# iamwinter/UMPR

Hardware: AMD Instinct MI355X
Metric: training samples/sec (higher is better)
Workload: dtype f32

## Files before the change

### include/umpr_hip.h

```cpp
#ifndef UMPR_HIP_H
#define UMPR_HIP_H
#include <stddef.h>
#include <stdint.h>

#ifdef __cplusplus
extern "C" {
#endif

const char* umpr_version(void);
const char* umpr_last_error(void);
int umpr_device_info(int dev, char* name, int name_len, int* compute_units, size_t* hbm_bytes);

int umpr_gemm_f32(const float* A, long lda, int transA, const float* B, long ldb, int transB, float* C, long ldc,
                  int M, int N, int K, const float* bias, int bias_mode, int act, int accumulate, float alpha,
                  float* ws, size_t ws_bytes, void* stream);

int umpr_set_gemm_bf16(int on);

int umpr_set_conv_inference(int on);

int umpr_set_conv_pool_follows(int on);

long umpr_debug_wino_fix_count(void);

size_t umpr_embed_gru_bidir_ws_bytes(int N, int L, int E);
int umpr_embed_gru_bidir_fwd(const int64_t* ids, const float* emb, int E,
                             const float* w_ih_f, const float* w_hh_f, const float* b_ih_f, const float* b_hh_f,
                             const float* w_ih_r, const float* w_hh_r, const float* b_ih_r, const float* b_hh_r,
                             const int32_t* lengths, const int32_t* order, const int32_t* dst_row, int N, int L,
                             float* out, float* saved, float* ws, size_t ws_bytes, void* stream);
int umpr_embed_gru_bidir_bwd(const int64_t* ids, const float* emb, int E,
                             const float* w_hh_f, const float* w_hh_r,
                             const int32_t* lengths, const int32_t* order, const int32_t* dst_row, int N, int L,
                             const float* dout, const float* out, const float* saved,
                             float* dw_ih_f, float* dw_hh_f, float* db_ih_f, float* db_hh_f,
                             float* dw_ih_r, float* dw_hh_r, float* db_ih_r, float* db_hh_r,
                             float* ws, size_t ws_bytes, void* stream);

int umpr_embed_gru_bidir_bwd_acc(const int64_t* ids, const float* emb, int E,
                                 const float* w_hh_f, const float* w_hh_r,
                                 const int32_t* lengths, const int32_t* order, const int32_t* dst_row, int N, int L,
                                 const float* dout, const float* out, const float* saved,
                                 float* dw_ih_f, float* dw_hh_f, float* db_ih_f, float* db_hh_f,
                                 float* dw_ih_r, float* dw_hh_r, float* db_ih_r, float* db_hh_r,
                                 int accumulate, float* ws, size_t ws_bytes, void* stream);

size_t umpr_coattention_fwd_ws_bytes(int B, int SL);
int umpr_coattention_fwd(const float* Gu, const float* Gi, const float* M, int B, int SL, float* T, float* soft_u,
                         float* soft_i, float* atte_u, long ld_u, float* atte_i, long ld_i, float* colmax,
                         int32_t* argcol, float* rowmax, int32_t* argrow, float* ws, size_t ws_bytes, void* stream);
int umpr_coattention_fwd_bf16(const float* Gu, const float* Gi, const float* M, int B, int SL, float* T, float* soft_u,
                              float* soft_i, float* atte_u, long ld_u, float* atte_i, long ld_i, float* colmax,
                              int32_t* argcol, float* rowmax, int32_t* argrow, float* ws, size_t ws_bytes, void* stream);
size_t umpr_coattention_bwd_ws_bytes(int B, int SL);
int umpr_coattention_bwd(const float* Gu, const float* Gi, const float* M, const float* T, const float* soft_u,
                         const float* soft_i, const float* colmax, const int32_t* argcol, const float* rowmax,
// ... 190 lines not shown
```

### umpr_amd/_lib.py

```python
from __future__ import annotations

import ctypes
import os
import threading

import torch

_HERE = os.path.dirname(os.path.abspath(__file__))
LIB_PATH = os.path.join(_HERE, "libumpr_hip.so")

_T = {"p": ctypes.c_void_p, "i": ctypes.c_int, "l": ctypes.c_long, "z": ctypes.c_size_t, "f": ctypes.c_float,
      "d": ctypes.c_double, "u": ctypes.c_uint64}

SIGNATURES = {
    "umpr_version": ("", "s"),
    "umpr_last_error": ("", "s"),
    "umpr_device_info": ("ipipp", "i"),
    "umpr_gemm_f32": ("pliplipliiipiiifpzp", "i"),
    "umpr_embed_gru_bidir_ws_bytes": ("iii", "z"),
    "umpr_embed_gru_bidir_fwd": ("ppipppppppppppiipppzp", "i"),
    "umpr_embed_gru_bidir_bwd": ("ppipppppiippppppppppppzp", "i"),
    "umpr_embed_gru_bidir_bwd_acc": ("ppipppppiipppppppppppipzp", "i"),
    "umpr_coattention_fwd_ws_bytes": ("ii", "z"),
    "umpr_coattention_fwd": ("pppiipppplplpppppzp", "i"),
# ... 51 lines not shown
    "umpr_vgg16_cls_arena_bytes": ("i", "z"),
    "umpr_vgg16_classifier_fwd_compact": ("piiiuppppzp", "i"),
    "umpr_vgg16_classifier_bwd_compact": ("piippppppzp", "i"),
    "umpr_vgg16_classifier_fwd_compact_bf16": ("piiiuppppzp", "i"),
    "umpr_vgg16_classifier_bwd_compact_bf16": ("piippppppzp", "i"),
    "umpr_concat_ids": ("pplpp", "i"),
    "umpr_review_net_arena_bytes": ("iii", "z"),
    "umpr_review_net_ws_bytes": ("iiii", "z"),
    "umpr_review_net_fwd": ("ppipppiiiiiipppzp", "i"),
    "umpr_review_net_bwd": ("ppipppiiiippppzp", "i"),
    "umpr_control_net_arena_bytes": ("iiiiiii", "z"),
    "umpr_control_net_ws_bytes": ("iiiiiiiii", "z"),
    "umpr_control_net_fwd": ("pppipppppiiiiiiiifiippppppzp", "i"),
    "umpr_control_net_bwd": ("pppipppppiiiiiiiiipppppppzp", "i"),
    "umpr_head_fwd": ("pppppppppppppfiiipppppppp", "i"),
    "umpr_head_bwd": ("pppppppppppfiiippppppppppppppppppppp", "i"),
    "umpr_photo_resize_u8": ("pzpiiipp", "i"),
    "umpr_photo_store_slot_bytes": ("ii", "z"),
    "umpr_photo_fetch_u8": ("pzpppiiiplpp", "i"),
    "umpr_bce_head_fwd": ("plpppiipppzp", "i"),
    "umpr_bce_head_bwd": ("plpppppiiplpppzp", "i"),
    "umpr_adam_step": ("ppppldddddldp", "i"),
    "umpr_sq_err_accumulate": ("pplpp", "i"),
    "umpr_adam_step_dev": ("pppplddd" "pp", "i"),
    "umpr_grad_norm_ws_bytes": ("", "z"),
    "umpr_grad_norm": ("ppidfppzpp", "i"),
    "umpr_adam_step_clip": ("ppppldddddld" "pp", "i"),
    "umpr_adam_step_dev_clip": ("pppplddd" "ppp", "i"),
    "umpr_debug_poison_lds": ("pp", "i"),
    "umpr_set_gemm_bf16": ("i", "i"),
    "umpr_set_conv_inference": ("i", "i"),
    "umpr_set_conv_pool_follows": ("i", "i"),
    "umpr_debug_wino_fix_count": ("", "l"),
    "umpr_profile_enable": ("i", "i"),
    "umpr_profile_reset": ("", "i"),
    "umpr_profile_read": ("ippp", "i"),
}


class UmprHipError(RuntimeError):
    pass


class _Tls(threading.local):
    gemm_b16 = False


TLS = _Tls()


class _Lib:
    def __init__(self):
        if not os.path.exists(LIB_PATH):
            raise UmprHipError(
                f"{LIB_PATH} not found: build it with `python -c 'import __graft_entry__ as g; g.build()'` "
                f"(or `make -C umpr_amd/csrc`).  There is no CPU fallback.")
        self.cdll = ctypes.CDLL(LIB_PATH)
        self.fn = {}
        for name, (args, ret) in SIGNATURES.items():
            f = getattr(self.cdll, name)
            f.argtypes = [_T[c] for c in args]
            f.restype = {"i": ctypes.c_int, "z": ctypes.c_size_t, "s": ctypes.c_char_p, "p": ctypes.c_void_p,
                         "l": ctypes.c_long}[ret]
            self.fn[name] = f

    def last_error(self) -> str:
# ... 55 lines not shown
```

### umpr_amd/csrc/api.hip

```cpp
#include <math.h>
#include <stdarg.h>
#include <stdlib.h>

#include <vector>

#include "../../include/umpr_hip.h"
#include "umpr_common.h"
#include "umpr_internal.h"

static thread_local char g_err[512] = "";
void umpr_set_error(const char* fmt, ...) {
  va_list ap;
  va_start(ap, fmt);
  vsnprintf(g_err, sizeof(g_err), fmt, ap);
  va_end(ap);
}

namespace {
const bool g_fc_small = umpr_env_on("UMPR_FC_SMALL");
const bool g_merge_small = umpr_env_on("UMPR_MERGE_SMALL");
struct ProfRec { hipEvent_t e0, e1; int family; double work; };
bool g_prof_on = false;
std::vector<ProfRec> g_prof;
std::vector<ProfRec> g_prof_pool;
// ... 57 lines not shown
  L.total = off;
  return L;
}
}

extern "C" {

const char* umpr_version(void) { return "umpr_hip 0.1 (gfx950)"; }
const char* umpr_last_error(void) { return g_err; }

int umpr_device_info(int dev, char* name, int name_len, int* compute_units, size_t* hbm_bytes) {
  hipDeviceProp_t prop;
  if (hipGetDeviceProperties(&prop, dev) != hipSuccess) { umpr_set_error("device_info: no device %d", dev); return -1; }
  if (name && name_len > 0) { strncpy(name, prop.name, name_len - 1); name[name_len - 1] = 0; }
  if (compute_units) *compute_units = prop.multiProcessorCount;
  if (hbm_bytes) *hbm_bytes = prop.totalGlobalMem;
  return 0;
}

int umpr_gemm_f32(const float* A, long lda, int transA, const float* B, long ldb, int transB, float* C, long ldc,
                  int M, int N, int K, const float* bias, int bias_mode, int act, int accumulate, float alpha,
                  float* ws, size_t ws_bytes, void* stream) {
  UmprGemm g;
  g.A = A; g.lda = lda; g.transA = transA != 0; g.B = B; g.ldb = ldb; g.transB = transB != 0; g.C = C; g.ldc = ldc;
  g.M = M; g.N = N; g.K = K; g.bias = bias; g.bias_mode = bias_mode; g.act = act; g.accumulate = accumulate != 0;
  g.alpha = alpha; g.split_k = ws ? 0 : 1; g.ws = ws; g.ws_bytes = ws_bytes;
  return umpr_gemm(g, S(stream));
}

int umpr_set_gemm_bf16(int on) { umpr_gemm_set_b16(on != 0); return 0; }
int umpr_set_conv_inference(int on) { umpr_wino_set_inference(on != 0); return 0; }
int umpr_set_conv_pool_follows(int on) { umpr_wino_set_pool_follows(on != 0); return 0; }
long umpr_debug_wino_fix_count(void) { return umpr_wino_last_fix_count(); }

constexpr size_t kSlabs = 256;
size_t umpr_embed_gru_bidir_ws_bytes(int N, int L, int E) {
  const size_t tiles = umpr_gru_tiles(N);
  const size_t Ep = (size_t)((E + 3) & ~3);
  return ((size_t)N * L * 384 + tiles * 2 * G3 * H + tiles * 2 * 2 * G3 + (size_t)kSlabs * G3 * Ep + (size_t)2 * G3 * Ep +
          (size_t)N * L * Ep) * sizeof(float);
}
namespace {
const bool g_emb_gather = umpr_env_on("UMPR_EMB_GATHER");
__global__ __launch_bounds__(256) void gather_rows_kernel(const int64_t* __restrict__ ids, const float* __restrict__ emb,
                                                          int E, int Ep, float* __restrict__ out, long rows) {
  const int lane = threadIdx.x & 63;
  for (long r = (long)blockIdx.x * 4 + (threadIdx.x >> 6); r < rows; r += (long)gridDim.x * 4) {
    const float* src = emb + ids[r] * (long)E;
    float* dst = out + r * (long)Ep;
    if ((E & 3) == 0) {
      for (int c = lane; c < E / 4; c += 64) reinterpret_cast<float4*>(dst)[c] = reinterpret_cast<const float4*>(src)[c];
    } else {
      for (int c = lane; c < Ep; c += 64) dst[c] = c < E ? src[c] : 0.f;
    }
  }
}
__global__ __launch_bounds__(256) void stack_wih_kernel(const float* __restrict__ wf, const float* __restrict__ wr,
                                                        const float* __restrict__ bf, const float* __restrict__ br, int E, int Ep,
                                                        float* __restrict__ wst, float* __restrict__ bst) {
  const int i = blockIdx.x * 256 + threadIdx.x;
  if (i < 2 * G3 * Ep) {
    const int row = i / Ep, c = i - row * Ep;
    const float* src = row < G3 ? wf + (long)row * E : wr + (long)(row - G3) * E;
    wst[i] = c < E ? src[c] : 0.f;
  }
  if (i < 2 * G3) bst[i] = i < G3 ? bf[i] : br[i - G3];
// ... 892 lines not shown
```

### umpr_amd/csrc/umpr_internal.h

```cpp
#pragma once
#include <hip/hip_runtime.h>
#include <stdint.h>

struct UmprGemm {
  const float* A = nullptr; long lda = 0; bool transA = false;
  const float* B = nullptr; long ldb = 0; bool transB = false;
  float* C = nullptr; long ldc = 0;
  int M = 0, N = 0, K = 0;
  const int64_t* gatherA = nullptr;
  const int64_t* gatherB = nullptr;
  const float* bias = nullptr; int bias_mode = 0;
  int act = 0; bool accumulate = false; float alpha = 1.0f;
  int split_k = 1;
  float* ws = nullptr; size_t ws_bytes = 0;
  int winA_L = 0, winA_D = 1, winA_pad = 0;
  int winB_L = 0, winB_D = 1, winB_pad = 0;
};
void umpr_gemm_set_b16(int on);
int umpr_gemm_b16();
int umpr_gemm(const UmprGemm& g, hipStream_t stream);

bool umpr_fc_small_ok(int M, int N, int K);
size_t umpr_fc_small_ws_bytes(int M, int N, int K);
int umpr_fc_small_fwd(const float* x, const float* W, const float* bias, float* out, int M, int N, int K, int act,
// ... 11 lines not shown
struct UmprHead {
  const float* rr;
  const float* c_u; const float* c_i; const float* pp; const float* pn;
  const float* vgg;
  const float* pos_v; const float* neg_v;
  const float* lw; const float* lb;
  const float* fw; const float* fb;
  const float* labels;
  float rate;
  int B, V, P, F;
  float* pred; float* loss;
  float* z;
  float* img_emb; float* pos_match; float* neg_match;
  float* posneg_emb;
  const float* d_loss;
  const float* d_pred;
  float* d_rr; float* d_cu; float* d_ci; float* d_pp; float* d_pn;
  float* d_vgg; float* d_pos_v; float* d_neg_v; float* d_lw; float* d_lb; float* d_fw; float* d_fb;
};
int umpr_head_launch(const UmprHead& p, int backward, hipStream_t s);

size_t umpr_conv3x3_pack_floats(int N, int Cin, int Cout, int H, int W);
int umpr_conv3x3_run(const float* x, const float* w, int transposed, const float* bias, const float* mask, float* y,
                     int N, int Cin, int Cout, int H, int W, int relu, float* wpack, size_t wpack_floats,
                     hipStream_t s);
size_t umpr_wino_ws_floats(int N, int C, int M, int H, int W, int transposed);
void umpr_wino_set_inference(int on);
void umpr_wino_set_pool_follows(int on);
long umpr_wino_last_fix_count();
void umpr_wino_set_v_slot(float* p, size_t floats);
size_t umpr_wino_v_floats(int N, int Cin, int Cout, int H, int W);
bool umpr_conv3x3_fwd_is_wino(int Cin, int Cout, int H, int W);
int umpr_wino_inference();
int umpr_wino_f4_mode();
size_t umpr_wino_wgrad_ws_floats(int N, int Cin, int Cout, int H, int W);
int umpr_wino_wgrad(const float* dy, const float* x, float* dw, float* db, int N, int Cin, int Cout, int H, int W,
                    int accumulate, float* ws, size_t ws_floats, hipStream_t s);
int umpr_wino_conv3x3(const float* x, const float* w, int transposed, const float* bias, const float* mask, float* y,
                      int N, int Cin, int Cout, int H, int W, int relu, float* ws, size_t ws_floats, hipStream_t s);
int umpr_conv3x3_flip_transpose(const float* w, float* wt, int Cout, int Cin, hipStream_t s);
size_t umpr_conv3x3_wgrad_ws_bytes(int N, int Cin, int Cout, int H, int W);
int umpr_conv3x3_wgrad(const float* gz, const float* x, float* dw, float* db, int N, int Cin, int Cout, int H, int W,
                       int accumulate, float* ws, size_t ws_bytes, hipStream_t s);
int umpr_maxpool2_fwd_impl(const float* x, float* y, long planes, int H, int W, hipStream_t s);
int umpr_maxpool2_bwd_relu_impl(const float* x, const float* gy, float* gx, long planes, int H, int W, hipStream_t s);

int umpr_wgrad_reduce(const float* slab, const float* bslab, int splits, int Cout, int Cin, float* dw, float* db,
                      int accumulate, hipStream_t s);

struct UmprPF {
  int N, H, W, RW;
  long rows;
  long ptot;
  long lead, tail;
  long ps;
};
UmprPF umpr_pf(int N, int H, int W);
size_t umpr_pf_bytes(const UmprPF& g, int C);
size_t umpr_conv_bf16_pack_bytes(int Cin, int Cout);
int umpr_conv_bf16_run(const void* x, const float* w, int transposed, const float* bias, const void* mask, void* y,
                       const UmprPF& g, int Cin, int Cout, int relu, void* wpack, size_t wpack_bytes, hipStream_t s,
                       bool zero_guards = true);
int umpr_conv_bf16_pack_all(const float* const* w, const int* Cin, const int* Cout, const int* W, int n, int transposed,
                            void* wpack, const size_t* offsets, hipStream_t s);
int umpr_pf_zero_guards_multi(void* const* bases, const UmprPF* geos, const int* channels, int n, hipStream_t s);
size_t umpr_wgrad_bf16_ws_bytes(const UmprPF& g, int Cin, int Cout);
// ... 91 lines not shown
```

### umpr_amd/csrc/winograd.hip

```cpp
#include <type_traits>

#include "umpr_common.h"
#include "umpr_internal.h"

namespace {

constexpr int WK = 32;
constexpr int WBM = 128;
constexpr int WBN = 128;
constexpr int WLDA = WBM + 4;

__global__ void wino_weights_kernel(const float* __restrict__ w, float* __restrict__ U, int M, int C, int CinW,
                                    int transposed) {
  const int MT = (M + WBM - 1) / WBM, S = (C + WK - 1) / WK;
  const long total = (long)MT * WBM * S * WK;
  for (long i = blockIdx.x * (long)blockDim.x + threadIdx.x; i < total; i += (long)gridDim.x * blockDim.x) {
    const int ml = (int)(i % WBM);
    long r = i / WBM;
    const int k = (int)(r % WK); r /= WK;
    const int s = (int)(r % S);
    const int mt = (int)(r / S);
    const int m = mt * WBM + ml, c = s * WK + k;
    float g[9];
#pragma unroll
    for (int t = 0; t < 9; ++t) {
      float v = 0.f;
      if (m < M && c < C) v = transposed ? w[((long)c * CinW + m) * 9 + 8 - t] : w[((long)m * CinW + c) * 9 + t];
      g[t] = v;
    }
    float gg[4][3];
#pragma unroll
    for (int j = 0; j < 3; ++j) {
// ... 562 lines not shown
#pragma unroll
      for (int dy = 0; dy < 3; ++dy) {
        const int py = yy + dy - 1;
        if (py < 0 || py >= H) continue;
#pragma unroll
        for (int dx = 0; dx < 3; ++dx) {
          const int px = xx + dx - 1;
          if (px < 0 || px >= W) continue;
          acc = fmaf(xp[(long)py * W + px], wp[dy * 3 + dx], acc);
        }
      }
    }
#pragma unroll
    for (int o = 32; o > 0; o >>= 1) acc += __shfl_xor(acc, o, 64);
    if (lane == 0) {
      float v = acc + (bias ? bias[m] : 0.f);
      if (relu) v = fmaxf(v, 0.f);
      y[idx] = v;
    }
  }
}

static long wino_tpad(long T) { return (T + WBN - 1) / WBN * WBN; }

struct WinoGemmParams {
  const float* U;
  const float* V;
  float* Mx;
  int MT, S, C;
  long Tpad;
  long TT;
  int Mpad;
  int planes;
};

__global__ __launch_bounds__(256, 2) void wino_gemm_kernel(WinoGemmParams p) {
  constexpr int LDA = WLDA, LDB = WBN;
  constexpr int TM = 2, TN = 2;
  constexpr int KS = WK / 2;
  constexpr int NV = 4;
  constexpr int SFLUSH = 4;
  __shared__ __attribute__((aligned(16))) float As[2][WK * LDA];
  __shared__ __attribute__((aligned(16))) float Bs[2][WK * LDB];
  const int tid = threadIdx.x, lane = tid & 63, wave = tid >> 6;
  const int wm = wave >> 1, wn = wave & 1;
  const int l31 = lane & 31, half = lane >> 5;
  const long TT = p.TT;
  const int xcd = blockIdx.x & 7;
  const long qq = blockIdx.x >> 3;
  const int mt = (int)(qq % p.MT);
  const long bt = (qq / p.MT) * 8 + xcd;
  if (bt >= p.planes * TT) return;
  const int xi = (int)(bt / TT);
  const long t0 = (bt % TT) * WBN;
  const float* Ub = p.U + (((long)xi * p.MT + mt) * p.S) * (WK * WBM);
  const float* Vb = p.V + (long)xi * (p.S * WK) * p.Tpad + t0;

  const float* pa = Ub + 4 * tid;
  const float* pb = Vb + (long)(tid >> 5) * p.Tpad + 4 * (tid & 31);
  const long bstep = 8 * p.Tpad;
  float* sa = &As[0][(tid >> 5) * LDA + 4 * (tid & 31)];
  float* sb = &Bs[0][(tid >> 5) * LDB + 4 * (tid & 31)];
  float4 ra0, ra1, ra2, ra3, rb0, rb1, rb2, rb3;
  auto lda = [&](int v, int s) { return *reinterpret_cast<const float4*>(pa + (long)s * (WK * WBM) + 1024 * v); };
  auto ldb = [&](int v, int s) { return *reinterpret_cast<const float4*>(pb + (long)s * 4 * bstep + v * bstep); };
  auto sta = [&](int v, int buf, const float4& r) { *reinterpret_cast<float4*>(sa + buf * (WK * LDA) + 8 * v * LDA) = r; };
  auto stb = [&](int v, int buf, const float4& r) { *reinterpret_cast<float4*>(sb + buf * (WK * LDB) + 8 * v * LDB) = r; };
  auto piece = [&](int q, int sn, int nbuf) {
    switch (q) {
      case 0: ra0 = lda(0, sn); break;
      case 1: ra1 = lda(1, sn); break;
      case 2: ra2 = lda(2, sn); break;
      case 3: ra3 = lda(3, sn); break;
      case 4: rb0 = ldb(0, sn); break;
      case 5: rb1 = ldb(1, sn); break;
      case 6: rb2 = ldb(2, sn); break;
      case 7: rb3 = ldb(3, sn); break;
      case 8: sta(0, nbuf, ra0); break;
      case 9: sta(1, nbuf, ra1); break;
      case 10: sta(2, nbuf, ra2); break;
      case 11: sta(3, nbuf, ra3); break;
      case 12: stb(0, nbuf, rb0); break;
      case 13: stb(1, nbuf, rb1); break;
      case 14: stb(2, nbuf, rb2); break;
      default: stb(3, nbuf, rb3); break;
    }
  };
// ... 50 lines not shown
      }
      __syncthreads();
    }
#pragma unroll
    for (int i = 0; i < TM; ++i)
#pragma unroll
      for (int j = 0; j < TN; ++j) tot[i][j] += acc[i][j];
  }
  float* Mb = p.Mx + ((long)xi * p.Mpad + mt * WBM) * p.Tpad + t0;
#pragma unroll
  for (int i = 0; i < TM; ++i)
#pragma unroll
    for (int j = 0; j < TN; ++j)
#pragma unroll
      for (int r = 0; r < 16; ++r)
        Mb[(long)(wm * 64 + i * 32 + mfma_row(r, lane)) * p.Tpad + wn * 64 + j * 32 + l31] = tot[i][j][r];
}

typedef __attribute__((address_space(3))) void* lds_ptr_t;
template <int SK, int OCC, int FOLD>
__global__ __launch_bounds__(256, OCC) void wino_gemm_dma_kernel(WinoGemmParams p) {
  constexpr int LD = 128;
  constexpr int TM = 2, TN = 2;
  constexpr int KS = SK / 2;
  constexpr int NP = SK / 8;
  constexpr int SFLUSH = FOLD == 0 ? 128 / SK : 1;
  typedef typename std::conditional<FOLD == 2, double, float>::type tot_t;
  __shared__ __attribute__((aligned(1024))) float As[2][SK * LD];
  __shared__ __attribute__((aligned(1024))) float Bs[2][SK * LD];
  const int tid = threadIdx.x, lane = tid & 63;
  const int wave = __builtin_amdgcn_readfirstlane(tid >> 6);
  const int wm = wave >> 1, wn = wave & 1;
  const int l31 = lane & 31, half = lane >> 5;
  const long TT = p.TT;
  const int xcd = blockIdx.x & 7;
  const long qq = blockIdx.x >> 3;
  const int mt = (int)(qq % p.MT);
  const long bt = (qq / p.MT) * 8 + xcd;
  if (bt >= p.planes * TT) return;
  const int xi = (int)(bt / TT);
  const long t0 = (bt % TT) * WBN;
  const float* Ub = p.U + (((long)xi * p.MT + mt) * p.S) * (WK * WBM);
  const float* Vb = p.V + (long)xi * (p.S * WK) * p.Tpad + t0;
  const float* ga = Ub + wave * (NP * 256) + lane * 4;
  const float* gb = Vb + (long)(wave * (2 * NP) + half) * p.Tpad + l31 * 4;
  const long bstep = 2 * p.Tpad;
  const unsigned lds_a = (unsigned)(size_t)(lds_ptr_t)(&As[0][0]) + (unsigned)wave * (NP * 1024u);
  const unsigned lds_b = (unsigned)(size_t)(lds_ptr_t)(&Bs[0][0]) + (unsigned)wave * (NP * 1024u);
  auto glds = [&](const float* src, unsigned dst) {
    unsigned keep;
    asm volatile("s_mov_b32 %0, m0\n\ts_mov_b32 m0, %2\n\ts_nop 0\n\tglobal_load_lds_dwordx4 %1, off\n\ts_mov_b32 m0, %0"
                 : "=&s"(keep) : "v"(src), "s"(dst) : "memory");
  };
  auto dma = [&](int q, int sn, int nbuf) {
    if (q < NP) glds(ga + (long)sn * (SK * WBM) + q * 256, lds_a + (unsigned)nbuf * (SK * LD * 4u) + (unsigned)q * 1024u);
    else glds(gb + (long)sn * SK * p.Tpad + (q - NP) * bstep, lds_b + (unsigned)nbuf * (SK * LD * 4u) + (unsigned)(q - NP) * 1024u);
  };
  auto dma_wait = [&]() { asm volatile("s_waitcnt vmcnt(0)" ::: "memory"); };

  f32x16 acc[TM][TN];
  tot_t tot[TM][TN][16];
#pragma unroll
  for (int i = 0; i < TM; ++i)
#pragma unroll
    for (int j = 0; j < TN; ++j)
#pragma unroll
      for (int r = 0; r < 16; ++r) { acc[i][j][r] = 0.f; tot[i][j][r] = (tot_t)0; }

  const int ns = p.S * (WK / SK);
#pragma unroll
  for (int q = 0; q < 2 * NP; ++q) dma(q, 0, 0);
  dma_wait();
  __syncthreads();
  for (int s0 = 0; s0 < ns; s0 += SFLUSH) {
// ... 25 lines not shown
          if (m == 0 && k1 < KS) {
#pragma unroll
            for (int ii = 0; ii < TM; ++ii) a[nb][ii] = as[2 * k1 * LD + ii * 32];
          }
          if (m == 1 && k1 < KS) {
#pragma unroll
            for (int jj = 0; jj < TN; ++jj) b[nb][jj] = bs[2 * k1 * LD + jj * 32];
          }
          if (m == 3 && kk < 2 * NP) dma(kk, sn, cur ^ 1);
          __builtin_amdgcn_sched_barrier(0);
        }
      }
      dma_wait();
      __syncthreads();
    }
#pragma unroll
    for (int i = 0; i < TM; ++i)
#pragma unroll
      for (int j = 0; j < TN; ++j)
#pragma unroll
        for (int r = 0; r < 16; ++r) tot[i][j][r] += (tot_t)acc[i][j][r];
  }
  float* Mb = p.Mx + ((long)xi * p.Mpad + mt * WBM) * p.Tpad + t0;
#pragma unroll
  for (int i = 0; i < TM; ++i)
#pragma unroll
    for (int j = 0; j < TN; ++j)
#pragma unroll
      for (int r = 0; r < 16; ++r)
        Mb[(long)(wm * 64 + i * 32 + mfma_row(r, lane)) * p.Tpad + wn * 64 + j * 32 + l31] = (float)tot[i][j][r];
}

const int g_wino_dma = umpr_env_int("UMPR_WINO_DMA", 1);

inline int nblk(long n, int cap) {
  long b = (n + 255) / 256;
  if (b > cap) b = cap;
  return (int)(b < 1 ? 1 : b);
}

}

int umpr_wino_f4_mode() {
  static const int mode = umpr_env_int("UMPR_WINO_F4", 2);
  return mode;
}
static thread_local int t_wino_infer = 0;
void umpr_wino_set_inference(int on) { t_wino_infer = on; }
int umpr_wino_inference() { return t_wino_infer && umpr_wino_f4_mode() >= 1; }
static inline bool wino_f4_shape(int H, int W) {
  return 36L * ((H + 3) / 4) * ((W + 3) / 4) < 16L * (H / 2) * (W / 2);
}
static thread_local int t_wino_pool_follows = 0;
void umpr_wino_set_pool_follows(int on) { t_wino_pool_follows = on; }
static thread_local float* t_v_slot = nullptr;
static thread_local size_t t_v_slot_floats = 0;
void umpr_wino_set_v_slot(float* p, size_t floats) { t_v_slot = p; t_v_slot_floats = floats; }

static thread_local const unsigned int* t_last_fix_count = nullptr;
long umpr_wino_last_fix_count() {
  if (!t_last_fix_count) return -1;
  unsigned int v = 0;
  if (hipDeviceSynchronize() != hipSuccess || hipMemcpy(&v, t_last_fix_count, sizeof(v), hipMemcpyDeviceToHost) != hipSuccess) return -2;
  return (long)v;
}
static inline bool wino_f4_map(int H, int W, int transposed) {
  const int need = transposed || t_wino_infer ? 1 : 2;
  return umpr_wino_f4_mode() >= need && wino_f4_shape(H, W);
}

size_t umpr_wino_ws_floats(int N, int C, int M, int H, int W, int transposed) {
  const long MT = (M + WBM - 1) / WBM, S = (C + WK - 1) / WK;
  auto layout = [&](bool f4) {
    const long T = f4 ? (long)N * ((H + 3) / 4) * ((W + 3) / 4) : (long)N * (H / 2) * (W / 2);
    const long Tpad = wino_tpad(T);
    return (size_t)(f4 ? 36 : 16) * (MT * WBM * S * WK + S * WK * Tpad + MT * WBM * Tpad) + 64 + (f4 ? Tpad : 0);
  };
  const bool map4 = wino_f4_shape(H, W);
  const int mode = umpr_wino_f4_mode();
// ... 72 lines not shown
  const long TT = (T + WBN - 1) / WBN;
  static const int kappa = umpr_env_int("UMPR_WINO_FIX_KAPPA", 8);
  const bool fix = f4 && !transposed && !t_wino_infer && kappa > 0 && mask == nullptr;
  WinoFix fx{nullptr, nullptr, 0u, 0.f, nullptr};
  unsigned int* tie_bits = nullptr;
  if (fix) {
    fx.count = reinterpret_cast<unsigned int*>(Mx + (size_t)planes * MT * WBM * Tpad);
    fx.list = reinterpret_cast<unsigned int*>(list_region);
    const size_t vfl = (size_t)planes * S * WK * Tpad;
    fx.cap = (unsigned)(vfl < (size_t)0x7fffffff ? vfl : (size_t)0x7fffffff);
    fx.kappa_eps = (float)kappa * 5.9604644775390625e-08f;
    UMPR_REQUIRE((long)N * M * H * W < 0xffffffffL, "winograd fix-up: output tensor too large for 32-bit element indices");
    if (t_wino_pool_follows) {
      tie_bits = fx.count + 16;
      if (hipMemsetAsync(tie_bits - 1, 0, (size_t)(T + 1) * sizeof(unsigned int), s) != hipSuccess) { umpr_set_error("winograd fix-up: memset"); return -2; }
      UMPR_REQUIRE(((long)N * C * H * W) % 4 == 0 && (reinterpret_cast<uintptr_t>(x) & 15) == 0, "winograd fix-up: unaligned input");
      wino_absmax_kernel<<<nblk((long)N * C * H * W / 4, 1024), 256, 0, s>>>(x, (long)N * C * H * W / 4, tie_bits - 1);
      UMPR_LAUNCH_CHECK("wino_absmax");
      fx.tie_bits = tie_bits;
    }
  }
  if (f4 && edge) {
    if (tie_bits) wino4_input_kernel<true, true><<<nblk((long)S * WK * TT * WBN, 16384), 256, 0, s>>>(x, V, N, C, S * WK, H, W, Tpad, TT * WBN, wino4_consts(), fx.count, tie_bits);
    else wino4_input_kernel<true, false><<<nblk((long)S * WK * TT * WBN, 16384), 256, 0, s>>>(x, V, N, C, S * WK, H, W, Tpad, TT * WBN, wino4_consts(), fx.count, nullptr);
  } else if (f4) {
    if (tie_bits) wino4_input_kernel<false, true><<<nblk((long)S * WK * TT * WBN, 16384), 256, 0, s>>>(x, V, N, C, S * WK, H, W, Tpad, TT * WBN, wino4_consts(), fx.count, tie_bits);
    else wino4_input_kernel<false, false><<<nblk((long)S * WK * TT * WBN, 16384), 256, 0, s>>>(x, V, N, C, S * WK, H, W, Tpad, TT * WBN, wino4_consts(), fx.count, nullptr);
  }
  else if ((W / 2) % 2 == 0)
    wino_input_pair_kernel<<<nblk((long)S * WK * TT * WBN / 2, 16384), 256, 0, s>>>(x, V, N, C, S * WK, H, W, Tpad, TT * WBN);
  else
    wino_input_kernel<<<nblk((long)S * WK * TT * WBN, 16384), 256, 0, s>>>(x, V, N, C, S * WK, H, W, Tpad, TT * WBN);
  UMPR_LAUNCH_CHECK("wino_input");
  WinoGemmParams p{U, V, Mx, MT, S, C, Tpad, TT, MT * WBM, planes};
  const long groups = (planes * TT + 7) / 8 * 8;
  {
    UmprProfScope prof(UMPR_K_WINO_GEMM, 2.0 * planes * (double)M * C * T, s);
    static const int fold = umpr_env_int("UMPR_WINO_FOLD", 1);
    if (g_wino_dma == 2) wino_gemm_dma_kernel<16, 3, 0><<<(unsigned)(groups * MT), 256, 0, s>>>(p);
    else if (g_wino_dma && fold == 2) wino_gemm_dma_kernel<32, 2, 2><<<(unsigned)(groups * MT), 256, 0, s>>>(p);
    else if (g_wino_dma && fold == 1) wino_gemm_dma_kernel<32, 2, 1><<<(unsigned)(groups * MT), 256, 0, s>>>(p);
    else if (g_wino_dma) wino_gemm_dma_kernel<32, 2, 0><<<(unsigned)(groups * MT), 256, 0, s>>>(p);
    else wino_gemm_kernel<<<(unsigned)(groups * MT), 256, 0, s>>>(p);
  }
  UMPR_LAUNCH_CHECK("wino_gemm");
  if (f4 && fix) {
    if (edge) wino4_output_kernel<true, true><<<nblk((long)M * T, 16384), 256, 0, s>>>(Mx, bias, mask, y, N, M, H, W, Tpad, MT * WBM, relu, wino4_consts(), fx);
    else wino4_output_kernel<false, true><<<nblk((long)M * T, 16384), 256, 0, s>>>(Mx, bias, mask, y, N, M, H, W, Tpad, MT * WBM, relu, wino4_consts(), fx);
    UMPR_LAUNCH_CHECK("wino_output");
    wino_fixup_kernel<<<128, 256, 0, s>>>(x, w, bias, y, fx.list, fx.count, fx.cap, C, M, H, W, relu);
    UMPR_LAUNCH_CHECK("wino_fixup");
    t_last_fix_count = fx.count;
    return 0;
  }
  if (f4 && edge)
    wino4_output_kernel<true, false><<<nblk((long)M * T, 16384), 256, 0, s>>>(Mx, bias, mask, y, N, M, H, W, Tpad, MT * WBM, relu, wino4_consts(), fx);
  else if (f4)
    wino4_output_kernel<false, false><<<nblk((long)M * T, 16384), 256, 0, s>>>(Mx, bias, mask, y, N, M, H, W, Tpad, MT * WBM, relu, wino4_consts(), fx);
  else if ((W / 2) % 2 == 0)
    wino_output_pair_kernel<<<nblk((long)M * T / 2, 16384), 256, 0, s>>>(Mx, bias, mask, y, N, M, H, W, Tpad, MT * WBM, relu);
  else
    wino_output_kernel<<<nblk((long)M * T, 16384), 256, 0, s>>>(Mx, bias, mask, y, N, M, H, W, Tpad, MT * WBM, relu);
  UMPR_LAUNCH_CHECK("wino_output");
  return 0;
}

namespace {

// ... 248 lines not shown
  if (g == 0 && ok) {
#pragma unroll
    for (int a = 0; a < 36; ++a) v[a] = ((v[a] + red[0][a][cl]) + red[1][a][cl]) + red[2][a][cl];
    float gv[3][6];
#pragma unroll
    for (int b = 0; b < 6; ++b) {
      float o[3];
      wino4_gt(wc, v + b, 6, o);
      gv[0][b] = o[0]; gv[1][b] = o[1]; gv[2][b] = o[2];
    }
#pragma unroll
    for (int a = 0; a < 3; ++a) {
      float o[3];
      wino4_gt(wc, gv[a], 1, o);
      outs[cl * 9 + a * 3 + 0] = o[0]; outs[cl * 9 + a * 3 + 1] = o[1]; outs[cl * 9 + a * 3 + 2] = o[2];
    }
  }
  __syncthreads();
  const int c0 = (blockIdx.x % chunks) * 64;
  const int nout = (C - c0 < 64 ? C - c0 : 64) * 9;
  float* d = dw + ((long)m * C + c0) * 9;
  for (int i = threadIdx.x; i < nout; i += 256) d[i] = accumulate ? d[i] + outs[i] : outs[i];
}

struct WinoWgradParams {
  const float* Gy;
  const float* V;
  float* P;
  int MT, CT, Mpad, Cpad;
  long Tpad;
  int stages;
  int stages_per_split;
  int planes;
};

constexpr int WLDK = WK + 4;

template <int TN>
__global__ __launch_bounds__(256, 2) void wino_wgrad_gemm_kernel(WinoWgradParams p) {
  constexpr int LD = WLDK;
  constexpr int TM = 2;
  constexpr int BNC = 64 * TN;
  constexpr int NG = WK / 8;
  constexpr int SFLUSH = 4;
  __shared__ __attribute__((aligned(16))) float As[2][WBM * LD];
  __shared__ __attribute__((aligned(16))) float Bs[2][BNC * LD];
  const int tid = threadIdx.x, lane = tid & 63, wave = tid >> 6;
  const int wm = wave >> 1, wn = wave & 1;
  const int l31 = lane & 31, half = lane >> 5;
  long b = blockIdx.x;
  const int ct = (int)(b % p.CT); b /= p.CT;
  const int mt = (int)(b % p.MT); b /= p.MT;
  const int xi = (int)(b % p.planes);
  const int split = (int)(b / p.planes);
  const int s_begin = split * p.stages_per_split;
  const int s_end = min(p.stages, s_begin + p.stages_per_split);
  const int ns = s_end - s_begin;

  const int urow = tid >> 3, uq = tid & 7;
  const float* pa = p.Gy + ((long)xi * p.Mpad + mt * WBM + urow) * p.Tpad + (long)s_begin * WK + 4 * uq;
  const float* pb = p.V + ((long)xi * p.Cpad + ct * BNC + urow) * p.Tpad + (long)s_begin * WK + 4 * uq;
  const long rstep = 32 * p.Tpad;
  float* sa = &As[0][urow * LD + 4 * uq];
  float* sb = &Bs[0][urow * LD + 4 * uq];
  float4 ra0, ra1, ra2, ra3, rb0, rb1, rb2, rb3;
  auto lda = [&](int v, int s) { return *reinterpret_cast<const float4*>(pa + (long)s * WK + v * rstep); };
  auto ldb = [&](int v, int s) { return *reinterpret_cast<const float4*>(pb + (long)s * WK + v * rstep); };
  auto sta = [&](int v, int buf, const float4& r) { *reinterpret_cast<float4*>(sa + buf * (WBM * LD) + 32 * v * LD) = r; };
  auto stb = [&](int v, int buf, const float4& r) { *reinterpret_cast<float4*>(sb + buf * (BNC * LD) + 32 * v * LD) = r; };
  auto piece = [&](int q, int sn, int nbuf) {
    switch (q) {
      case 0: ra0 = lda(0, sn); break;
      case 1: ra1 = lda(1, sn); break;
      case 2: ra2 = lda(2, sn); break;
      case 3: ra3 = lda(3, sn); break;
      case 4: rb0 = ldb(0, sn); break;
      case 5: rb1 = ldb(1, sn); break;
      case 6: if (TN == 2) rb2 = ldb(2, sn); break;
      case 7: if (TN == 2) rb3 = ldb(3, sn); break;
      case 8: sta(0, nbuf, ra0); break;
      case 9: sta(1, nbuf, ra1); break;
      case 10: sta(2, nbuf, ra2); break;
      case 11: sta(3, nbuf, ra3); break;
// ... 175 lines not shown
  const WinoWgradGeom g = wino_wgrad_geom(N, Cin, Cout, H, W);
  float* Gy = ws;
  float* V = Gy + (size_t)g.planes * g.Mpad * g.Tpad;
  float* P = V + (size_t)g.planes * g.Cpad * g.Tpad;
  float* BP = P + (size_t)g.planes * g.splits * g.Mpad * g.Cpad;
  const bool f4 = g.planes == 36;
  const bool edge = f4 && ((H % 4) != 0 || (W % 4) != 0);
  static const bool bias_fuse = umpr_env_on("UMPR_WINO_BIAS_FUSE");
  const bool fused_bias = db && f4 && !edge && bias_fuse && (g.Tpad % 64) == 0;
  if (f4 && edge)
    wino4_dy_kernel<true><<<nblk((long)Cout * g.Tpad, 16384), 256, 0, s>>>(dy, Gy, N, Cout, H, W, g.Tpad, g.Tpad, g.Mpad, wino4_consts(), nullptr);
  else if (f4)
    wino4_dy_kernel<false><<<nblk((long)Cout * g.Tpad, 16384), 256, 0, s>>>(dy, Gy, N, Cout, H, W, g.Tpad, g.Tpad, g.Mpad, wino4_consts(),
                                                                            fused_bias ? BP : nullptr);
  else if ((W / 2) % 2 == 0)
    wino_dy_pair_kernel<<<nblk((long)Cout * g.Tpad / 2, 16384), 256, 0, s>>>(dy, Gy, N, Cout, H, W, g.Tpad, g.Tpad, g.Mpad);
  else
    wino_dy_kernel<<<nblk((long)Cout * g.Tpad, 16384), 256, 0, s>>>(dy, Gy, N, Cout, H, W, g.Tpad, g.Tpad, g.Mpad);
  UMPR_LAUNCH_CHECK("wino_dy");
  if (t_v_slot) {
    const size_t vfl = umpr_wino_v_floats(N, Cin, Cout, H, W);
    UMPR_REQUIRE(f4 && !edge && vfl == (size_t)g.planes * g.Cpad * g.Tpad && t_v_slot_floats >= vfl,
                 "winograd wgrad: the V slot does not match this layer (%d -> %d at %dx%d)", Cin, Cout, H, W);
    V = t_v_slot;
  } else if (f4 && edge)
    wino4_input_kernel<true, false><<<nblk((long)g.Cpad * g.Tpad, 16384), 256, 0, s>>>(x, V, N, Cin, g.Cpad, H, W, g.Tpad, g.Tpad, wino4_consts(), nullptr, nullptr);
  else if (f4)
    wino4_input_kernel<false, false><<<nblk((long)g.Cpad * g.Tpad, 16384), 256, 0, s>>>(x, V, N, Cin, g.Cpad, H, W, g.Tpad, g.Tpad, wino4_consts(), nullptr, nullptr);
  else if ((W / 2) % 2 == 0)
    wino_input_pair_kernel<<<nblk((long)g.Cpad * g.Tpad / 2, 16384), 256, 0, s>>>(x, V, N, Cin, g.Cpad, H, W, g.Tpad, g.Tpad);
  else
    wino_input_kernel<<<nblk((long)g.Cpad * g.Tpad, 16384), 256, 0, s>>>(x, V, N, Cin, g.Cpad, H, W, g.Tpad, g.Tpad);
  UMPR_LAUNCH_CHECK("wino_input(wgrad)");
  WinoWgradParams p{Gy, V, P, g.MT, g.CT, g.Mpad, g.Cpad, g.Tpad, g.stages, g.stages_per_split, g.planes};
  {
    UmprProfScope prof(UMPR_K_WINO_WGRAD_GEMM, 2.0 * g.planes * (double)Cout * Cin * g.T, s);
    if (g.bnc == 64) wino_wgrad_gemm_kernel<1><<<(unsigned)(g.planes * g.MT * g.CT * g.splits), 256, 0, s>>>(p);
    else wino_wgrad_gemm_kernel<2><<<(unsigned)(g.planes * g.MT * g.CT * g.splits), 256, 0, s>>>(p);
  }
  UMPR_LAUNCH_CHECK("wino_wgrad_gemm");
  if (f4)
    wino4_wgrad_finish_kernel<<<(unsigned)((long)Cout * ((Cin + 63) / 64)), 256, 0, s>>>(P, g.splits, Cout, Cin, g.Mpad, g.Cpad, dw,
                                                                                     accumulate, wino4_consts());
  else if (g.splits >= 8)
    wino_wgrad_finish_wide_kernel<<<(unsigned)((long)Cout * ((Cin + 63) / 64)), 256, 0, s>>>(P, g.splits, Cout, Cin, g.Mpad, g.Cpad,
                                                                                         dw, accumulate);
  else
    wino_wgrad_finish_kernel<<<nblk((long)Cout * Cin, 4096), 256, 0, s>>>(P, g.splits, Cout, Cin, g.Mpad, g.Cpad, dw, accumulate);
  UMPR_LAUNCH_CHECK("wino_wgrad_finish");
  if (fused_bias) {
    wino_bias_sum_waves_kernel<<<(unsigned)((Cout + 3) / 4), 256, 0, s>>>(BP, db, Cout, g.Tpad / 64, accumulate);
    UMPR_LAUNCH_CHECK("wino_bias_sum_waves");
  } else if (db) {
    UMPR_REQUIRE((size_t)N * Cout <= (size_t)g.splits * g.planes * g.Mpad * g.Cpad && ((long)H * W) % 4 == 0,
                 "winograd wgrad: bias-gradient scratch");
    wino_bias_part_wave_kernel<<<(unsigned)(((long)N * Cout + 3) / 4), 256, 0, s>>>(dy, P, (long)H * W, (long)N * Cout);
    UMPR_LAUNCH_CHECK("wino_bias_part");
    wino_bias_sum_kernel<<<(Cout + 255) / 256, 256, 0, s>>>(P, db, N, Cout, accumulate);
    UMPR_LAUNCH_CHECK("wino_bias_sum");
  }
  return 0;
}
```

Measured before the change: 2083.

## Remap Winograd GEMM block order so each XCD reuses the same plane's tiles

Changes how block indices are decoded in the Winograd forward GEMM and weight-gradient GEMM. Blocks that share a plane, and so share U/Gy operand tiles, are placed on the same XCD (blockIdx & 7) so they hit that XCD's L2. The forward path switches to segmented ordering only when the estimated U working set exceeds a 2 MB budget. The wgrad path groups all MT*CT tiles of a plane/split onto one XCD when there are 64 or fewer. This adds padded grids with early-exit blocks and a runtime toggle, at the cost of some tail imbalance.

After: 2081. No clear change (-0.1%).

```diff
diff --git a/include/umpr_hip.h b/include/umpr_hip.h
--- a/include/umpr_hip.h
+++ b/include/umpr_hip.h
@@ -22,6 +22,8 @@
 int umpr_set_conv_pool_follows(int on);
 
 long umpr_debug_wino_fix_count(void);
+
+int umpr_wino_set_xcd_order(int on);
 
 size_t umpr_embed_gru_bidir_ws_bytes(int N, int L, int E);
 int umpr_embed_gru_bidir_fwd(const int64_t* ids, const float* emb, int E,
diff --git a/umpr_amd/_lib.py b/umpr_amd/_lib.py
--- a/umpr_amd/_lib.py
+++ b/umpr_amd/_lib.py
@@ -107,6 +107,7 @@
     "umpr_set_conv_inference": ("i", "i"),
     "umpr_set_conv_pool_follows": ("i", "i"),
     "umpr_debug_wino_fix_count": ("", "l"),
+    "umpr_wino_set_xcd_order": ("i", "i"),
     "umpr_profile_enable": ("i", "i"),
     "umpr_profile_reset": ("", "i"),
     "umpr_profile_read": ("ippp", "i"),
diff --git a/umpr_amd/csrc/api.hip b/umpr_amd/csrc/api.hip
--- a/umpr_amd/csrc/api.hip
+++ b/umpr_amd/csrc/api.hip
@@ -113,6 +113,7 @@
 int umpr_set_conv_inference(int on) { umpr_wino_set_inference(on != 0); return 0; }
 int umpr_set_conv_pool_follows(int on) { umpr_wino_set_pool_follows(on != 0); return 0; }
 long umpr_debug_wino_fix_count(void) { return umpr_wino_last_fix_count(); }
+int umpr_wino_set_xcd_order(int on) { return umpr_wino_xcd_order_exchange(on); }
 
 constexpr size_t kSlabs = 256;
 size_t umpr_embed_gru_bidir_ws_bytes(int N, int L, int E) {
diff --git a/umpr_amd/csrc/umpr_internal.h b/umpr_amd/csrc/umpr_internal.h
--- a/umpr_amd/csrc/umpr_internal.h
+++ b/umpr_amd/csrc/umpr_internal.h
@@ -67,6 +67,7 @@
 size_t umpr_wino_v_floats(int N, int Cin, int Cout, int H, int W);
 bool umpr_conv3x3_fwd_is_wino(int Cin, int Cout, int H, int W);
 int umpr_wino_inference();
+int umpr_wino_xcd_order_exchange(int on);
 int umpr_wino_f4_mode();
 size_t umpr_wino_wgrad_ws_floats(int N, int Cin, int Cout, int H, int W);
 int umpr_wino_wgrad(const float* dy, const float* x, float* dw, float* db, int N, int Cin, int Cout, int H, int W,
diff --git a/umpr_amd/csrc/winograd.hip b/umpr_amd/csrc/winograd.hip
--- a/umpr_amd/csrc/winograd.hip
+++ b/umpr_amd/csrc/winograd.hip
@@ -1,3 +1,4 @@
+#include <atomic>
 #include <type_traits>
 
 #include "umpr_common.h"
@@ -626,7 +627,27 @@
   long TT;
   int Mpad;
   int planes;
+  int nseg;
+  int seg_len;
 };
+
+__device__ __forceinline__ bool wino_gemm_decode(const WinoGemmParams& p, int& mt, int& xi, long& tcol) {
+  const int xcd = blockIdx.x & 7;
+  const long qq = blockIdx.x >> 3;
+  mt = (int)(qq % p.MT);
+  const long r = qq / p.MT;
+  if (p.nseg == 0) {
+    const long bt = r * 8 + xcd;
+    if (bt >= p.planes * p.TT) return false;
+    xi = (int)(bt / p.TT);
+    tcol = bt % p.TT;
+    return true;
+  }
+  const long unit = (r / p.seg_len) * 8 + xcd;
+  xi = (int)(unit / p.nseg);
+  tcol = (unit % p.nseg) * p.seg_len + r % p.seg_len;
+  return tcol < p.TT;
+}
 
 __global__ __launch_bounds__(256, 2) void wino_gemm_kernel(WinoGemmParams p) {
   constexpr int LDA = WLDA, LDB = WBN;
@@ -639,14 +660,10 @@
   const int tid = threadIdx.x, lane = tid & 63, wave = tid >> 6;
   const int wm = wave >> 1, wn = wave & 1;
   const int l31 = lane & 31, half = lane >> 5;
-  const long TT = p.TT;
-  const int xcd = blockIdx.x & 7;
-  const long qq = blockIdx.x >> 3;
-  const int mt = (int)(qq % p.MT);
-  const long bt = (qq / p.MT) * 8 + xcd;
-  if (bt >= p.planes * TT) return;
-  const int xi = (int)(bt / TT);
-  const long t0 = (bt % TT) * WBN;
+  int mt, xi;
+  long tcol;
+  if (!wino_gemm_decode(p, mt, xi, tcol)) return;
+  const long t0 = tcol * WBN;
   const float* Ub = p.U + (((long)xi * p.MT + mt) * p.S) * (WK * WBM);
   const float* Vb = p.V + (long)xi * (p.S * WK) * p.Tpad + t0;
 
@@ -763,14 +780,10 @@
   const int wave = __builtin_amdgcn_readfirstlane(tid >> 6);
   const int wm = wave >> 1, wn = wave & 1;
   const int l31 = lane & 31, half = lane >> 5;
-  const long TT = p.TT;
-  const int xcd = blockIdx.x & 7;
-  const long qq = blockIdx.x >> 3;
-  const int mt = (int)(qq % p.MT);
-  const long bt = (qq / p.MT) * 8 + xcd;
-  if (bt >= p.planes * TT) return;
-  const int xi = (int)(bt / TT);
-  const long t0 = (bt % TT) * WBN;
+  int mt, xi;
+  long tcol;
+  if (!wino_gemm_decode(p, mt, xi, tcol)) return;
+  const long t0 = tcol * WBN;
   const float* Ub = p.U + (((long)xi * p.MT + mt) * p.S) * (WK * WBM);
   const float* Vb = p.V + (long)xi * (p.S * WK) * p.Tpad + t0;
   const float* ga = Ub + wave * (NP * 256) + lane * 4;
@@ -862,6 +875,8 @@
 }
 
 const int g_wino_dma = umpr_env_int("UMPR_WINO_DMA", 1);
+std::atomic<int> g_wino_xcd_order{umpr_env_int("UMPR_WINO_XCD_ORDER", 1)};
+constexpr long kWinoUBudgetBytes = 2L << 20;
 
 inline int nblk(long n, int cap) {
   long b = (n + 255) / 256;
@@ -875,6 +890,7 @@
   static const int mode = umpr_env_int("UMPR_WINO_F4", 2);
   return mode;
 }
+int umpr_wino_xcd_order_exchange(int on) { return g_wino_xcd_order.exchange(on != 0); }
 static thread_local int t_wino_infer = 0;
 void umpr_wino_set_inference(int on) { t_wino_infer = on; }
 int umpr_wino_inference() { return t_wino_infer && umpr_wino_f4_mode() >= 1; }
@@ -1013,8 +1029,14 @@
   else
     wino_input_kernel<<<nblk((long)S * WK * TT * WBN, 16384), 256, 0, s>>>(x, V, N, C, S * WK, H, W, Tpad, TT * WBN);
   UMPR_LAUNCH_CHECK("wino_input");
-  WinoGemmParams p{U, V, Mx, MT, S, C, Tpad, TT, MT * WBM, planes};
-  const long groups = (planes * TT + 7) / 8 * 8;
+  WinoGemmParams p{U, V, Mx, MT, S, C, Tpad, TT, MT * WBM, planes, 0, 0};
+  long groups = (planes * TT + 7) / 8 * 8;
+  if (g_wino_xcd_order && (128 / TT + 1) * (long)MT * WBM * S * WK * 4 > kWinoUBudgetBytes) {
+    p.nseg = planes % 8 == 0 ? 1 : planes % 4 == 0 ? 2 : planes % 2 == 0 ? 4 : 8;
+    p.seg_len = (int)((TT + p.nseg - 1) / p.nseg);
+    groups = (long)planes * p.nseg * p.seg_len;
+  }
+  UMPR_REQUIRE(groups * MT < 0x7fffffffL, "winograd: GEMM grid too large");
   {
     UmprProfScope prof(UMPR_K_WINO_GEMM, 2.0 * planes * (double)M * C * T, s);
     static const int fold = umpr_env_int("UMPR_WINO_FOLD", 1);
@@ -1329,6 +1351,7 @@
   int stages;
   int stages_per_split;
   int planes;
+  int xcd_groups;
 };
 
 constexpr int WLDK = WK + 4;
@@ -1346,6 +1369,13 @@
   const int wm = wave >> 1, wn = wave & 1;
   const int l31 = lane & 31, half = lane >> 5;
   long b = blockIdx.x;
+  if (p.xcd_groups) {
+    const int G = p.MT * p.CT;
+    const long q = b >> 3;
+    const long group = (q / G) * 8 + (b & 7);
+    if (group >= p.xcd_groups) return;
+    b = group * G + q % G;
+  }
   const int ct = (int)(b % p.CT); b /= p.CT;
   const int mt = (int)(b % p.MT); b /= p.MT;
   const int xi = (int)(b % p.planes);
@@ -1587,11 +1617,18 @@
   else
     wino_input_kernel<<<nblk((long)g.Cpad * g.Tpad, 16384), 256, 0, s>>>(x, V, N, Cin, g.Cpad, H, W, g.Tpad, g.Tpad);
   UMPR_LAUNCH_CHECK("wino_input(wgrad)");
-  WinoWgradParams p{Gy, V, P, g.MT, g.CT, g.Mpad, g.Cpad, g.Tpad, g.stages, g.stages_per_split, g.planes};
+  WinoWgradParams p{Gy, V, P, g.MT, g.CT, g.Mpad, g.Cpad, g.Tpad, g.stages, g.stages_per_split, g.planes, 0};
+  const int G = g.MT * g.CT, ngroups = g.planes * g.splits;
+  long blocks = (long)ngroups * G;
+  if (g_wino_xcd_order && G > 1 && G <= 64) {
+    p.xcd_groups = ngroups;
+    blocks = 8L * G * ((ngroups + 7) / 8);
+  }
+  UMPR_REQUIRE(blocks < 0x7fffffffL, "winograd wgrad: GEMM grid too large");
   {
     UmprProfScope prof(UMPR_K_WINO_WGRAD_GEMM, 2.0 * g.planes * (double)Cout * Cin * g.T, s);
-    if (g.bnc == 64) wino_wgrad_gemm_kernel<1><<<(unsigned)(g.planes * g.MT * g.CT * g.splits), 256, 0, s>>>(p);
-    else wino_wgrad_gemm_kernel<2><<<(unsigned)(g.planes * g.MT * g.CT * g.splits), 256, 0, s>>>(p);
+    if (g.bnc == 64) wino_wgrad_gemm_kernel<1><<<(unsigned)blocks, 256, 0, s>>>(p);
+    else wino_wgrad_gemm_kernel<2><<<(unsigned)blocks, 256, 0, s>>>(p);
   }
   UMPR_LAUNCH_CHECK("wino_wgrad_gemm");
   if (f4)
```
